# RoozbehSanaei/Structure-from-Motion-3D-Reconstruction

Measured on AMD Instinct MI355X. Metric: keyframes/sec (KLT + RANSAC + local BA per-frame loop), synthetic TempleRing-47 stand-in, higher is better.
Workload: dtype f64

## Files before the change

### include/sfmx.h

```cpp
#ifndef SFMX_H
#define SFMX_H

#include <stdint.h>

#ifdef __cplusplus
extern "C" {
#endif

typedef enum sfmx_status {
  SFMX_OK = 0,
  SFMX_ERR_INVALID = 1,
  SFMX_ERR_HIP = 2,
  SFMX_ERR_NO_DEVICE = 3,
  SFMX_ERR_SINGULAR = 4,
  SFMX_ERR_UNSUPPORTED = 5
} sfmx_status;

typedef struct sfmx_ctx sfmx_ctx;
typedef struct sfmx_pyramid sfmx_pyramid;

int sfmx_ctx_create(int device_id, sfmx_ctx** out);
int sfmx_ctx_create_prio(int device_id, int priority, sfmx_ctx** out);
void sfmx_ctx_destroy(sfmx_ctx* ctx);
const char* sfmx_last_error(const sfmx_ctx* ctx);
// ... 39 lines not shown
int sfmx_ransac_score_ex(sfmx_ctx* ctx, const double* xi, const double* xj, int n, const int32_t* idx8,
                         int H, double thr, int32_t* counts_out, int32_t* lo_out, int32_t* hi_out,
                         uint8_t* flags_out, double* cond_out, int32_t* best_iter,
                         int32_t* best_count, double* E_out);
int sfmx_ransac_score(sfmx_ctx* ctx, const double* xi, const double* xj, int n, const int32_t* idx8,
                      int H, double thr, int32_t* counts_out, int32_t* best_iter, int32_t* best_count,
                      double* E_out);
int sfmx_sampson_mask(sfmx_ctx* ctx, const double* xi, const double* xj, int n, const double* E9,
                      double thr, uint8_t* mask_out, int32_t* count_out);

typedef struct sfmx_ba_problem sfmx_ba_problem;
int sfmx_ba_create(sfmx_ctx* ctx, int W, int P, const double* X, const int32_t* obs_ptr,
                   const int32_t* obs_li, const double* obs_uv, sfmx_ba_problem** out);
int sfmx_ba_reset(sfmx_ctx* ctx, sfmx_ba_problem* prob, int W, int P, const double* X, const int32_t* obs_ptr,
                  const int32_t* obs_li, const double* obs_uv);
void sfmx_ba_destroy(sfmx_ctx* ctx, sfmx_ba_problem* prob);
int sfmx_ba_build(sfmx_ctx* ctx, sfmx_ba_problem* prob, const double* poses_wc, double fx, double fy,
                  double cx, double cy, double huber, double lambda, int damp, double* S_out,
                  double* b_out);
int sfmx_ba_step(sfmx_ctx* ctx, sfmx_ba_problem* prob, const double* poses_wc, double fx, double fy,
                 double cx, double cy, double huber, double lambda, double* dx_out);
int sfmx_ba_begin(sfmx_ctx* ctx, sfmx_ba_problem* prob, int iters, double fx, double fy, double cx, double cy, double huber,
                  double lambda);
int sfmx_ba_end(sfmx_ctx* ctx, sfmx_ba_problem* prob);
int sfmx_ba_build_partial(sfmx_ctx* ctx, sfmx_ba_problem* prob, const double* poses_wc, double fx,
                          double fy, double cx, double cy, double huber, void** S_dev, void** b_dev);

typedef struct sfmx_comm sfmx_comm;
#define SFMX_COMM_ID_BYTES 128
int sfmx_comm_get_unique_id(void* id_out);
// ... 463 lines not shown
```

### structure-from-motion-3d-reconstruction_amd/capi.py

```python
from __future__ import annotations

import ctypes
import os
from ctypes import POINTER, byref, c_char_p, c_double, c_int, c_int32, c_uint8, c_uint32, c_uint64, c_void_p

import numpy as np

os.environ.setdefault("GPU_MAX_HW_QUEUES", "8")

_HERE = os.path.dirname(os.path.abspath(__file__))
LIB_PATH = os.path.join(_HERE, "_build", "libsfmx.so")

SFMX_OK, SFMX_ERR_INVALID, SFMX_ERR_HIP, SFMX_ERR_NO_DEVICE, SFMX_ERR_SINGULAR, SFMX_ERR_UNSUPPORTED = range(6)

SYMBOLS = [
    "sfmx_ctx_create", "sfmx_ctx_create_prio", "sfmx_ctx_destroy", "sfmx_last_error", "sfmx_sync", "sfmx_ctx_device", "sfmx_ctx_make_current", "sfmx_stream", "sfmx_set_timing", "sfmx_get_timing",
    "sfmx_last_kernel_us", "sfmx_kernel_profile", "sfmx_kernel_profile_name", "sfmx_pyramid_create", "sfmx_pyramid_destroy", "sfmx_pyramid_upload",
    "sfmx_pyramid_set_device", "sfmx_pyramid_set_device_async", "sfmx_pyramid_wait", "sfmx_pyramid_fetched_level", "sfmx_pyramid_download_level", "sfmx_pyramid_level_size", "sfmx_shi_tomasi_score",
    "sfmx_shi_tomasi_candidates", "sfmx_shi_tomasi_candidates_pruned", "sfmx_shi_tomasi_fetch_all_keys", "sfmx_klt_track", "sfmx_ransac_score", "sfmx_ransac_score_ex", "sfmx_sampson_mask", "sfmx_ba_create",
    "sfmx_ba_reset", "sfmx_ba_destroy", "sfmx_ba_build", "sfmx_ba_step", "sfmx_ba_begin", "sfmx_ba_end", "sfmx_ba_build_partial", "sfmx_ba_step_sharded", "sfmx_ba_step_sharded_elements", "sfmx_solve_dense", "sfmx_posegraph_solve",
    "sfmx_comm_get_unique_id", "sfmx_comm_create", "sfmx_comm_destroy", "sfmx_comm_rank", "sfmx_comm_world", "sfmx_shard_range",
    "sfmx_comm_allreduce_f64", "sfmx_comm_allreduce_u64_max",
    "sfmx_debug_hypot", "sfmx_debug_divsqrt", "sfmx_debug_klt_slow_steps",
    "sfmx_stereo_default_params", "sfmx_stereo_check_params", "sfmx_stereo_create", "sfmx_stereo_destroy", "sfmx_stereo_disparity",
    "sfmx_stereo_last_us",
    "sfmx_fusion_default_params", "sfmx_fusion_check_params", "sfmx_fusion_create", "sfmx_fusion_destroy", "sfmx_fusion_reset",
    "sfmx_fusion_add_view", "sfmx_fusion_add_stereo_view", "sfmx_fusion_integrate", "sfmx_fusion_read", "sfmx_fusion_extract",
    "sfmx_fusion_last_us",
    "sfmx_fusion_extract_normals", "sfmx_fusion_normals_us",
    "sfmx_shade_default_params", "sfmx_shade_check_params", "sfmx_shade_create", "sfmx_shade_destroy", "sfmx_shade_reset",
    "sfmx_shade_add_view", "sfmx_shade_add_stereo_view", "sfmx_shade_view_count", "sfmx_shade_vertices", "sfmx_shade_fusion",
    "sfmx_shade_last_us",
    "sfmx_consist_default_params", "sfmx_consist_check_params", "sfmx_consist_create", "sfmx_consist_destroy", "sfmx_consist_reset",
    "sfmx_consist_add_view", "sfmx_consist_add_stereo_view", "sfmx_consist_view_count", "sfmx_consist_filter", "sfmx_consist_read",
    "sfmx_consist_counts", "sfmx_fusion_add_consist_view", "sfmx_consist_last_us",
# ... 2117 lines not shown
        obs_uv = _f64(obs_uv)
        self.P = X.shape[0]
        self.h_ = c_void_p()
        ctx._chk(ctx.lib.sfmx_ba_create(ctx.h_, c_int(W), c_int(self.P), _p(X, c_double), _p(obs_ptr, c_int32),
                                        _p(obs_li, c_int32), _p(obs_uv, c_double), byref(self.h_)))

    def reset(self, W: int, X, obs_ptr, obs_li, obs_uv):
        X = _f64(X)
        obs_ptr = np.ascontiguousarray(obs_ptr, np.int32)
        obs_li = np.ascontiguousarray(obs_li, np.int32)
        obs_uv = _f64(obs_uv)
        self.ctx._chk(self.ctx.lib.sfmx_ba_reset(self.ctx.h_, self.h_, c_int(W), c_int(X.shape[0]), _p(X, c_double), _p(obs_ptr, c_int32),
                                                 _p(obs_li, c_int32), _p(obs_uv, c_double)))
        self.W, self.P = W, X.shape[0]

    def build(self, poses_wc, fx, fy, cx, cy, huber, lam, damp=True):
        D = 6 * self.W
        poses = _f64(poses_wc)
        S = np.zeros((D, D))
        b = np.zeros(D)
        self.ctx._chk(self.ctx.lib.sfmx_ba_build(self.ctx.h_, self.h_, _p(poses, c_double), c_double(fx), c_double(fy),
                                                 c_double(cx), c_double(cy), c_double(huber), c_double(lam),
                                                 c_int(1 if damp else 0), _p(S, c_double), _p(b, c_double)))
        return S, b

    def step(self, poses_wc, fx, fy, cx, cy, huber, lam):
        poses = _f64(poses_wc)
        dx = np.zeros(6 * self.W)
        rc = self.ctx.lib.sfmx_ba_step(self.ctx.h_, self.h_, _p(poses, c_double), c_double(fx), c_double(fy), c_double(cx),
                                       c_double(cy), c_double(huber), c_double(lam), _p(dx, c_double))
# ... 305 lines not shown
```

### structure-from-motion-3d-reconstruction_amd/csrc/hip/ba.hip

```cpp
#include "sfmx_internal.h"

#include <chrono>
#include <cstdio>
#include <cstdlib>
#include <mutex>
#include <vector>

#ifdef SFMX_BA_WGSTAMPS
#define WGS_CAP (1u << 20)
__device__ unsigned long long g_wgs_ring[WGS_CAP][8];
__device__ unsigned g_wgs_next;
struct WgStamp {
  unsigned long long t0, m[4] = {0, 0, 0, 0};
  unsigned hw;
  __device__ __forceinline__ void mark(int i) { m[i] = __builtin_amdgcn_s_memrealtime(); }
  __device__ __forceinline__ WgStamp() {
    t0 = __builtin_amdgcn_s_memrealtime();
    hw = (unsigned)__builtin_amdgcn_s_getreg((31 << 11) | 4) | ((unsigned)__builtin_amdgcn_s_getreg((3 << 11) | 20) << 28);
  }
  __device__ __forceinline__ void done(int kind, int blk, int nblk) const {
    __syncthreads();
    if (threadIdx.x == 0) {
      const unsigned slot = atomicAdd(&g_wgs_next, 1u) & (WGS_CAP - 1);
      g_wgs_ring[slot][0] = t0;
// ... 27 lines not shown
#define WGS_BEGIN
#define WGS_END(kind, blk, nblk)
#define WGS_MARK(i)
#define WGS_PARAM
#define WGS_ARG
#endif

#define BA_SLOT 84
#define BA_MAX_OBS 16
#define BA_MAX_W 64

struct sfmx_ba_problem {
  int W = 0, P = 0, R = 0, MS = 0;
  DevBuf bufs[12];
  double* X = nullptr;
  int32_t* obs_ptr = nullptr;
  int32_t* obs_li = nullptr;
  double* obs_uv = nullptr;
  double* poses = nullptr;
  double* rec = nullptr;
  int8_t* slot_of = nullptr;
  double* S = nullptr;
  double* b = nullptr;
  double* work = nullptr;
  double* contrib = nullptr;
  unsigned* ticket = nullptr;
  hipEvent_t ev_sync = nullptr, ev_exp[2] = {nullptr, nullptr}, ev_red[2] = {nullptr, nullptr};
  int chunk = 0;
  bool lds_points = false;
  bool job_active = false;
// ... 868 lines not shown
  }
  WGS_MARK(1);
  __syncthreads();
  if (tid < BAR_COLS && valid) {
    if (is_b) {
      if (damp && i < 6) acc = 0.0;
      b[i] = acc;
    } else {
      if (damp && i == j) {
        acc += lambda;
        if (i < 6) acc += 1e9;
      }
      S[(size_t)i * D + j] = acc;
    }
  }
  if constexpr (SOLVE_N > 0) {
    __shared__ int is_last;
    if (publish_system == 2) {
      if (tid < BAR_COLS && valid) {
        host_out[e] = acc;
        __threadfence_system();
      }
      __syncthreads();
      if (tid == 0) {
        const bool last = __hip_atomic_fetch_add(ticket, 1u, __ATOMIC_ACQ_REL, __HIP_MEMORY_SCOPE_AGENT) == (unsigned)nblk - 1u;
        if (last) {
          __hip_atomic_store(ticket, 0u, __ATOMIC_RELAXED, __HIP_MEMORY_SCOPE_AGENT);
          __threadfence_system();
          __hip_atomic_store(reinterpret_cast<unsigned long long*>(host_out + (SOLVE_N * SOLVE_N + SOLVE_N)), seq, __ATOMIC_RELEASE, __HIP_MEMORY_SCOPE_SYSTEM);
        }
      }
      WGS_MARK(2);
      return;
    }
    if (tid < BAR_COLS) __threadfence();
    __syncthreads();
    if (tid == 0) is_last = atomicAdd(ticket, 1u) == (unsigned)nblk - 1u ? 1 : 0;
    __syncthreads();
    WGS_MARK(2);
    if (!is_last) return;
    __threadfence();
    if (tid == 0) *ticket = 0;
    if (publish_system) {
      const int ne = SOLVE_N * SOLVE_N + SOLVE_N;
      for (int k = tid; k < ne; k += 256) host_out[k] = S[k];
      __threadfence_system();
      __syncthreads();
      if (tid == 0)
        __hip_atomic_store(reinterpret_cast<unsigned long long*>(host_out + ne), seq, __ATOMIC_RELEASE, __HIP_MEMORY_SCOPE_SYSTEM);
// ... 465 lines not shown
                             int publish_system, bool streaming) {
  const char* tile_env = getenv("SFMX_BA_TILE");
  const int tile_rows = tile_env ? atoi(tile_env) : 32;
  if (fused_solve && q->W == 6 && tile_rows == 32) {
    k_ba_reduce<32, 36, 4, 2><<<nwg, 256, 0, c->stream>>>(q->W, p_cnt, rows, lambda, damp, S_out, b_out, q->ticket, q->work, host_out, seq, wave_prio, init,
                                                         wg_lo, publish_system);
  } else if (fused_solve && q->W == 6 && tile_rows == 16) {
    k_ba_reduce<16, 36, 8, 2><<<nwg, 256, 0, c->stream>>>(q->W, p_cnt, rows, lambda, damp, S_out, b_out, q->ticket, q->work, host_out, seq, wave_prio, init,
                                                         wg_lo, publish_system);
  } else if (fused_solve && q->W == 6) {
    k_ba_reduce<64, 36, 2, 2><<<nwg, 256, 0, c->stream>>>(q->W, p_cnt, rows, lambda, damp, S_out, b_out, q->ticket, q->work, host_out, seq, wave_prio, init,
                                                         wg_lo, publish_system);
  } else if (fused_solve && q->W == 10) {
    k_ba_reduce<128, 60, 2, 2><<<nwg, 256, 0, c->stream>>>(q->W, p_cnt, rows, lambda, damp, S_out, b_out, q->ticket, q->work, host_out, seq, wave_prio, init,
                                                          wg_lo, publish_system);
  } else if (!streaming) {
    k_ba_reduce<64, 0, 2, 2><<<nwg, 256, 0, c->stream>>>(q->W, p_cnt, rows, lambda, damp, S_out, b_out, nullptr, nullptr, nullptr, 0, wave_prio, init, wg_lo);
  } else {
    k_ba_reduce<128, 0, 2, 2><<<nwg, 256, 0, c->stream>>>(q->W, p_cnt, rows, lambda, damp, S_out, b_out, nullptr, nullptr, nullptr, 0, wave_prio, init, wg_lo);
  }
}
static int ba_launch_reduce(sfmx_ctx* c, sfmx_ba_problem* q, int p_lo, int p_cnt, double lambda, int damp, double* S_out, double* b_out,
                            const double* init, bool fused_solve, double* host_out, unsigned long long seq, int wave_prio, int wg_lo = 0,
                            int wg_cnt = -1, int publish_system = 0, int e_lo = 0, int e_hi = 0x7fffffff) {
  const size_t CS = (size_t)36 * q->W * q->W + 48 * q->W;
  const int nwg = wg_cnt >= 0 ? wg_cnt : ba_element_blocks(q);
  if (nwg == 0 || p_cnt <= 0) return SFMX_OK;
  if (wg_cnt >= 0) fused_solve = false;
  if (q->chunk == 0) {
    SFMX_PROF(c, KID_BA_REDUCE, ba_reduce_kernel(c, q, q->contrib + (size_t)p_lo * CS, p_cnt, lambda, damp, S_out, b_out, init, fused_solve, host_out, seq,
// ... 106 lines not shown
  if (rc) return rc;
  for (int r = 0; r < n_ranks; ++r) {
    int lo = 0, hi = 0;
    sfmx_shard_range(q->P, r, n_ranks, &lo, &hi);
    if (order == 4) rc = ba_launch_reduce(c, q, lo, hi - lo, 0.0, 0, q->S, q->b, r == 0 ? nullptr : q->S, false, nullptr, 0, ba_wave_prio());
    else rc = ba_launch_reduce(c, q, lo, hi - lo, 0.0, 0, part + (size_t)r * NE, part + (size_t)r * NE + (size_t)D * D, nullptr, false, nullptr, 0,
                               ba_wave_prio());
    if (rc) return rc;
  }
  if (order != 4) k_ba_combine_partials<<<(NE + 255) / 256, 256, 0, c->stream>>>(part, n_ranks, NE, order, q->S);
  t.stop();
  SFMX_HIP(c, hipGetLastError());
  return SFMX_OK;
}

extern "C" {

int sfmx_ba_reset(sfmx_ctx* c, sfmx_ba_problem* q, int W, int P, const double* X, const int32_t* obs_ptr, const int32_t* obs_li,
                  const double* obs_uv) {
  SFMX_REQUIRE(c, c && q && W >= 1 && W <= BA_MAX_W && P >= 1 && X && obs_ptr && obs_li && obs_uv);
  if (q->job_active) (void)sfmx_ba_end(c, q);
  const int R = obs_ptr[P];
  SFMX_REQUIRE(c, R >= 0 && obs_ptr[0] == 0);
  q->W = W; q->P = P; q->R = R;
  q->MS = W < BA_MAX_OBS ? W : BA_MAX_OBS;
  const int D = 6 * W;
  const size_t CS = (size_t)36 * W * W + 36 * W + 12 * W;
  auto up16 = [](size_t v) { return (v + 15) & ~(size_t)15; };
  const size_t o_x = 0, o_uv = up16((size_t)P * 24), o_ptr = o_uv + up16((size_t)R * 16), o_li = o_ptr + up16((size_t)(P + 1) * 4);
  const size_t in_bytes = o_li + up16((size_t)R * 4) + 16;
  q->chunk = ba_merged(q) ? 0 : ba_chunk_points();
  const size_t row_slots = q->chunk ? (size_t)2 * q->chunk : (size_t)P;
  const size_t need[11] = {in_bytes, 16, 16, 16, (size_t)W * 96,
                           (size_t)P * q->MS * BA_SLOT * 8, (size_t)P * W, (size_t)D * D * 8 + (size_t)D * 8, 16, (size_t)D * 8 + 64,
                           row_slots * CS * 8};
  const void* ticket_before = q->bufs[8].p;
  for (int i = 0; i < 11; i++) SFMX_HIP(c, q->bufs[i].ensure(need[i]));
  const bool new_ticket = q->bufs[8].p != ticket_before;
  q->ticket = q->bufs[8].as<unsigned>();
  q->contrib = q->bufs[10].as<double>();
  char* in = q->bufs[0].as<char>();
  q->X = reinterpret_cast<double*>(in + o_x); q->obs_uv = reinterpret_cast<double*>(in + o_uv);
  q->obs_ptr = reinterpret_cast<int32_t*>(in + o_ptr); q->obs_li = reinterpret_cast<int32_t*>(in + o_li);
  q->poses = q->bufs[4].as<double>(); q->rec = q->bufs[5].as<double>();
  q->slot_of = q->bufs[6].as<int8_t>(); q->S = q->bufs[7].as<double>(); q->b = q->S + (size_t)D * D;
  q->work = q->bufs[9].as<double>();
  q->lds_points = false;
  if (ba_merged(q)) {
    bool dup = false;
    for (int p = 0; p < P && !dup; p++) {
      const int o0 = obs_ptr[p], cnt = obs_ptr[p + 1] - o0;
      if (cnt < 2 || cnt > BA_MAX_OBS) continue;
      unsigned long long seen = 0;
      for (int k = 0; k < cnt; k++) {
        const int li = obs_li[o0 + k];
        if (li < 0 || li >= W) continue;
        if (seen >> li & 1ull) { dup = true; break; }
        seen |= 1ull << li;
      }
    }
    q->lds_points = !dup;
  }
  if (c->ba_upload_in_flight) {
    SFMX_HIP(c, hipStreamSynchronize(c->stream));
    c->ba_upload_in_flight = false;
  }
  SFMX_HIP(c, c->h[4].ensure(in_bytes));
  char* st = c->h[4].as<char>();
  memcpy(st + o_x, X, (size_t)P * 24);
  memcpy(st + o_ptr, obs_ptr, (size_t)(P + 1) * 4);
  if (R > 0) {
    memcpy(st + o_uv, obs_uv, (size_t)R * 16);
    memcpy(st + o_li, obs_li, (size_t)R * 4);
  }
  SFMX_HIP(c, hipMemcpyAsync(in, st, in_bytes, hipMemcpyHostToDevice, c->stream));
  if (new_ticket) SFMX_HIP(c, hipMemsetAsync(q->ticket, 0, 16, c->stream));
  c->ba_upload_in_flight = true;
  return SFMX_OK;
}

int sfmx_ba_create(sfmx_ctx* c, int W, int P, const double* X, const int32_t* obs_ptr, const int32_t* obs_li, const double* obs_uv,
                   sfmx_ba_problem** out) {
  SFMX_REQUIRE(c, c && out);
  sfmx_ba_problem* q = new sfmx_ba_problem;
  const int rc = sfmx_ba_reset(c, q, W, P, X, obs_ptr, obs_li, obs_uv);
  if (rc != SFMX_OK) {
    sfmx_ba_destroy(c, q);
    return rc;
  }
  *out = q;
  return SFMX_OK;
}

void sfmx_ba_destroy(sfmx_ctx* c, sfmx_ba_problem* q) {
  if (!q) return;
  if (q->job_active && c) (void)sfmx_ba_end(c, q);
  if (c) { (void)hipStreamSynchronize(c->stream); (void)hipStreamSynchronize(c->copy_stream); }
  for (auto& b : q->bufs) b.release();
  q->job_ctl.release();
  q->job_cmd.release();
  if (q->ev_sync) (void)hipEventDestroy(q->ev_sync);
  for (int k = 0; k < 2; k++) {
    if (q->ev_exp[k]) (void)hipEventDestroy(q->ev_exp[k]);
    if (q->ev_red[k]) (void)hipEventDestroy(q->ev_red[k]);
  }
  delete q;
}

int sfmx_ba_build(sfmx_ctx* c, sfmx_ba_problem* q, const double* poses_wc, double fx, double fy, double cx, double cy, double huber,
                  double lambda, int damp, double* S_out, double* b_out) {
  SFMX_REQUIRE(c, c && q && poses_wc && S_out && b_out);
  KernelTimer t(c);
  int rc = ba_launch_build(c, q, poses_wc, fx, fy, cx, cy, huber, lambda, damp, t);
  if (rc) return rc;
  const int D = 6 * q->W;
  SFMX_HIP(c, hipMemcpyAsync(S_out, q->S, (size_t)D * D * 8, hipMemcpyDeviceToHost, c->stream));
  SFMX_HIP(c, hipMemcpyAsync(b_out, q->b, (size_t)D * 8, hipMemcpyDeviceToHost, c->stream));
  SFMX_HIP(c, hipStreamSynchronize(c->stream));
  c->ba_upload_in_flight = false;
  t.collect();
  return SFMX_OK;
}

int sfmx_ba_build_partial(sfmx_ctx* c, sfmx_ba_problem* q, const double* poses_wc, double fx, double fy, double cx, double cy,
                          double huber, void** S_dev, void** b_dev) {
  SFMX_REQUIRE(c, c && q && poses_wc && S_dev && b_dev);
  KernelTimer t(c);
  int rc = ba_launch_build(c, q, poses_wc, fx, fy, cx, cy, huber, 0.0, 0, t);
  if (rc) return rc;
  SFMX_HIP(c, hipStreamSynchronize(c->stream));
  c->ba_upload_in_flight = false;
  t.collect();
  *S_dev = q->S;
  *b_dev = q->b;
  return SFMX_OK;
}

extern "C" int sfmx_host_solve_window(const double* S, const double* b, int n, double* x, double* work);

int sfmx_ba_begin(sfmx_ctx* c, sfmx_ba_problem* q, int iters, double fx, double fy, double cx, double cy, double huber, double lambda) {
  SFMX_REQUIRE(c, c && q && iters >= 0);
  if (q->job_active) (void)sfmx_ba_end(c, q);
  const char* e = getenv("SFMX_BA_RESIDENT");
  const char* se = getenv("SFMX_BA_SOLVE");
  const bool off = !(e && e[0] == '1') || (se && std::string(se) == "device") || getenv("SFMX_BA_NO_POLL") || getenv("SFMX_BA_NO_FUSE");
  if (off || c->timing || iters < 1 || q->W != 6 || q->chunk != 0 || q->P > BA_MERGED_EXPAND_MAX_P) return SFMX_OK;
  const int D = 6 * q->W, NE = D * D + D;
  SFMX_HIP(c, q->job_ctl.ensure(sizeof(BaResidentCtl)));
  SFMX_HIP(c, q->job_cmd.ensure(16 * 8));
  q->job_slot = (q->job_slot + 1) & 15;
  SFMX_HIP(c, c->h[0].ensure((size_t)q->W * 96));
  SFMX_HIP(c, c->h[1].ensure((size_t)NE * 8 + 32));
  __atomic_store_n(q->job_cmd.as<unsigned long long>() + q->job_slot, 0ull, __ATOMIC_RELEASE);
  *reinterpret_cast<volatile unsigned long long*>(c->h[1].as<double>() + NE) = 0;
  SFMX_HIP(c, hipMemsetAsync(q->job_ctl.p, 0, sizeof(BaResidentCtl), c->stream));
  q->job_first_seq = c->ba_seq + 1;
// ... 33 lines not shown
      __atomic_store_n(q->job_cmd.as<unsigned long long>() + q->job_slot, BAW_EXIT, __ATOMIC_RELEASE);
      q->job_active = false;
      SFMX_HIP(c, hipStreamSynchronize(c->stream));
      return sfmx_fail(c, SFMX_ERR_HIP, "BA step result never arrived (resident kernel)", hipSuccess);
    }
  }
  q->job_done++;
  if (q->job_done >= q->job_iters) q->job_active = false;
  double work[36 * 37];
  const int status = sfmx_host_solve_window(hout, hout + (size_t)D * D, D, dx_out, work);
  return status ? SFMX_ERR_SINGULAR : SFMX_OK;
}

int sfmx_ba_step(sfmx_ctx* c, sfmx_ba_problem* q, const double* poses_wc, double fx, double fy, double cx, double cy, double huber,
                 double lambda, double* dx_out) {
  SFMX_REQUIRE(c, c && q && poses_wc && dx_out);
  if (q->job_active) {
    const double k[6] = {fx, fy, cx, cy, huber, lambda};
    if (memcmp(k, q->job_k, sizeof k) == 0 && !c->timing) return ba_step_resident(c, q, poses_wc, dx_out);
    (void)sfmx_ba_end(c, q);
  }
  const int D = 6 * q->W, NE = D * D + D;
  static const bool no_poll = getenv("SFMX_BA_NO_POLL") != nullptr;
  static const bool no_fuse = getenv("SFMX_BA_NO_FUSE") != nullptr;
  const char* solve_env = getenv("SFMX_BA_SOLVE");
  const bool host_solve_on = !(solve_env && std::string(solve_env) == "device");
  const bool poll = !c->timing && !no_poll;
  const bool fuse = ba_can_fuse_solve(q) && !no_fuse;
  const bool host_solve = host_solve_on && poll && fuse;
  static const bool host_times = getenv("SFMX_BA_HOST_TIMES") != nullptr;
  static double ht_launch = 0, ht_wait = 0, ht_solve = 0, ht_between = 0;
  static unsigned ht_n = 0;
  static std::chrono::steady_clock::time_point ht_last_exit;
  const auto ht0 = std::chrono::steady_clock::now();
  auto ht_us = [](std::chrono::steady_clock::time_point a, std::chrono::steady_clock::time_point b) { return std::chrono::duration<double, std::micro>(b - a).count(); };
  if (host_times && ht_n > 0 && ht_us(ht_last_exit, ht0) < 200.0) ht_between += ht_us(ht_last_exit, ht0);
  KernelTimer t(c);
  SFMX_HIP(c, c->h[1].ensure(host_solve ? (size_t)NE * 8 + 32 : (size_t)D * 8 + 32));
  double* hout = c->h[1].as<double>();
  volatile unsigned long long* flag = reinterpret_cast<volatile unsigned long long*>(host_solve ? hout + NE : hout + D + 1);
  const unsigned long long seq = ++c->ba_seq;
  if (poll) *flag = 0;
  const char* pub_env = getenv("SFMX_BA_PUBLISH");
  const int publish_mode = (pub_env && pub_env[0] == 'l') ? 1 : 2;
  int rc = ba_launch_build(c, q, poses_wc, fx, fy, cx, cy, huber, lambda, 1, t, poll, fuse, poll ? hout : nullptr, seq, host_solve ? publish_mode : 0);
  if (rc) return rc;
  if (!fuse) {
    int* dstatus = reinterpret_cast<int*>(q->work + D);
    rc = launch_solve(c, q->S, q->b, D, q->work, dstatus);
    if (rc) return rc;
  }
  int status = 0;
  if (poll) {
    if (!fuse) {
      k_ba_publish<<<1, 64, 0, c->stream>>>(q->work, D, hout, seq);
      SFMX_HIP(c, hipGetLastError());
    }
    const auto t0 = std::chrono::steady_clock::now();
    if (host_times) ht_launch += ht_us(ht0, t0);
    unsigned spins = 0;
// ... 17 lines not shown
        ht_solve += ht_us(ts, te);
        ht_last_exit = te;
        if (++ht_n == 1000) {
          fprintf(stderr, "[sfmx] ba step host times (us, mean of 1000): launches %.1f | wait for S|b %.1f | host solve %.1f | between steps %.1f\n", ht_launch / 1000,
                  ht_wait / 1000, ht_solve / 1000, ht_between / 1000);
          ht_launch = ht_wait = ht_solve = ht_between = 0;
          ht_n = 0;
        }
      }
      return status ? SFMX_ERR_SINGULAR : SFMX_OK;
    }
    memcpy(dx_out, hout, (size_t)D * 8);
    memcpy(&status, hout + D, 4);
    return status ? SFMX_ERR_SINGULAR : SFMX_OK;
  }
  SFMX_HIP(c, hipMemcpyAsync(c->h[1].p, q->work, (size_t)D * 8 + 4, hipMemcpyDeviceToHost, c->stream));
  SFMX_HIP(c, hipStreamSynchronize(c->stream));
  c->ba_upload_in_flight = false;
  t.collect();
  memcpy(dx_out, c->h[1].p, (size_t)D * 8);
  memcpy(&status, c->h[1].as<char>() + (size_t)D * 8, 4);
  return status ? SFMX_ERR_SINGULAR : SFMX_OK;
}

int sfmx_ba_step_sharded(sfmx_ctx* c, sfmx_comm* comm, sfmx_ba_problem* q, const double* poses_wc, double fx, double fy, double cx, double cy,
                         double huber, double lambda, double* dx_out) {
  SFMX_REQUIRE(c, c && q && poses_wc && dx_out);
  const int D = 6 * q->W;
  KernelTimer t(c);
  const int vworld = (!comm || comm->world <= 1) ? ba_virtual_world() : 0;
  int rc = (vworld > 1 && q->P >= vworld) ? ba_build_virtual_world(c, q, vworld, poses_wc, fx, fy, cx, cy, huber, t)
                                          : ba_launch_build(c, q, poses_wc, fx, fy, cx, cy, huber, 0.0, 0, t);
  if (rc) return rc;
  rc = sfmx_comm_allreduce_dev(c, comm, q->S, (size_t)D * D + D, 0, 0);
  if (rc) return rc;
  k_ba_damp_gauge<<<(D + 63) / 64, 64, 0, c->stream>>>(q->S, q->b, D, lambda);
  int* dstatus = reinterpret_cast<int*>(q->work + D);
  rc = launch_solve(c, q->S, q->b, D, q->work, dstatus);
  if (rc) return rc;
  int status = 0;
  SFMX_HIP(c, c->h[1].ensure((size_t)D * 8 + 8));
  SFMX_HIP(c, hipMemcpyAsync(c->h[1].p, q->work, (size_t)D * 8 + 4, hipMemcpyDeviceToHost, c->stream));
  SFMX_HIP(c, hipStreamSynchronize(c->stream));
  c->ba_upload_in_flight = false;
  t.collect();
  memcpy(dx_out, c->h[1].p, (size_t)D * 8);
  memcpy(&status, c->h[1].as<char>() + (size_t)D * 8, 4);
  return status ? SFMX_ERR_SINGULAR : SFMX_OK;
}

int sfmx_ba_step_sharded_elements(sfmx_ctx* c, sfmx_comm* comm, sfmx_ba_problem* q, const double* poses_wc, double fx, double fy, double cx,
                                  double cy, double huber, double lambda, double* dx_out) {
  SFMX_REQUIRE(c, c && q && poses_wc && dx_out);
  const int D = 6 * q->W, NE = D * D + D;
  const bool real = comm && comm->world > 1;
  const int vworld = real ? 0 : ba_virtual_world();
  const int world = real ? comm->world : (vworld > 1 ? vworld : 1);
  const int nblk = ba_element_blocks(q);
  KernelTimer t(c);
  int rc = SFMX_OK;
  const double* d_poses = ba_stage_poses(c, q, poses_wc, false, &rc);
  if (rc) return rc;
  double* part = nullptr;
  if (vworld > 1) {
    SFMX_HIP(c, q->bufs[11].ensure((size_t)vworld * NE * 8));
    part = q->bufs[11].as<double>();
    SFMX_HIP(c, hipMemsetAsync(part, 0, (size_t)vworld * NE * 8, c->stream));
  }
// ... 66 lines not shown
```

### structure-from-motion-3d-reconstruction_amd/csrc/host/pipeline.cpp

```cpp
#include "pipeline.hpp"

#include "../hip/sfmx_math.h"
#include "cli_io.hpp"
#include "stereo.hpp"
#include "introsort_replay.hpp"
#include "thread_pool.hpp"
#include "lane_plan.hpp"
#include "sfmx_ctx_split.h"
#pragma weak sfmx_ctx_create_bare
#pragma weak sfmx_ctx_create_stream

#include <algorithm>
#include <chrono>
#include <cmath>
#include <cstdio>
#include <cstdlib>
#include <cstring>
#include <filesystem>
#include <fstream>
#include <sstream>

namespace sfmx_host {

namespace {
// ... 837 lines not shown
  return job;
}

void GpuBundleAdjuster::gather_values(BaJob& job, const std::vector<Keyframe>& kfs, const V3* const* pending_xw) {
  if (job.P == 0) return;
  for (const auto& a : job.await) {
    const V3& x = *pending_xw[(size_t)a.second];
    job.X[(size_t)3 * a.first] = x.x; job.X[(size_t)3 * a.first + 1] = x.y; job.X[(size_t)3 * a.first + 2] = x.z;
  }
  job.await.clear();
  job.win.resize((size_t)job.W);
  for (int li = 0; li < job.W; li++) job.win[(size_t)li] = kfs[(size_t)(job.w0 + li)].pose;
  job.valid = true;
}

void GpuBundleAdjuster::solve(BaJob& job) {
  if (!job.valid) return;
  const auto t0 = Clock::now();
  const int W = job.W, P = job.P, D = 6 * W;
  const Mat3& K = job.K;
  const bool multi = comm_ && sfmx_comm_world(comm_) > 1;
  const char* vw = std::getenv("SFMX_VIRTUAL_WORLD");
  const bool virtual_world = !multi && vw && std::atoi(vw) > 1;
  const char* sm = std::getenv("SFMX_BA_SHARD");
  const bool by_points = sm && std::string(sm) == "points";
  const bool sharded = multi && by_points && P >= sfmx_comm_world(comm_);
  const bool by_elements = (multi || virtual_world) && !by_points;
  const double* Xp = job.X.data();
  const std::int32_t* optr = job.optr.data();
  const std::int32_t* oli = job.oli.data();
  const double* ouv = job.uv.data();
  int Pl = P;
  std::vector<std::int32_t> optr_local;
  if (sharded) {
    int lo = 0, hi = P;
    sfmx_shard_range(P, sfmx_comm_rank(comm_), sfmx_comm_world(comm_), &lo, &hi);
    Pl = hi - lo;
    const std::int32_t o0 = job.optr[(size_t)lo];
    optr_local.resize((size_t)Pl + 1);
    for (int p = 0; p <= Pl; p++) optr_local[(size_t)p] = job.optr[(size_t)(lo + p)] - o0;
    Xp += (size_t)3 * lo;
    optr = optr_local.data();
    oli += o0;
    ouv += (size_t)2 * o0;
  }
  if (!prob_) check(ctx_, sfmx_ba_create(ctx_, W, Pl, Xp, optr, oli, ouv, &prob_), "ba_create");
  else check(ctx_, sfmx_ba_reset(ctx_, prob_, W, Pl, Xp, optr, oli, ouv), "ba_reset");
  std::vector<double> poses((size_t)W * 12), dx((size_t)D);
  if (clk_) clk_->ba_calls++;
  const bool plain = !by_elements && !sharded && !virtual_world;
  struct JobGuard {
    sfmx_ctx* c; sfmx_ba_problem* q; bool on;
    ~JobGuard() { if (on) (void)sfmx_ba_end(c, q); }
  } job_guard{ctx_, prob_, false};
  if (plain) {
    check(ctx_, sfmx_ba_begin(ctx_, prob_, job.cfg.iters, K(0, 0), K(1, 1), K(0, 2), K(1, 2), job.cfg.huber_delta, job.cfg.lambda), "ba_begin");
    job_guard.on = true;
  }
  for (int it = 0; it < job.cfg.iters; ++it) {
    for (int li = 0; li < W; li++) {
      Mat3 R;
// ... 636 lines not shown
    const auto tj = Clock::now();
    if (lane_c) {
      if (pending_loop.active && pending_loop.ticket) lane_c->wait_ticket(pending_loop.ticket);
      else if (!queued_loop.active) lane_c->wait();
    }
    clk.join_wait += since(tj);
    if (pending_loop.active) {
      PendingLoop pl = pending_loop;
      pending_loop = PendingLoop{};
      if (pl.cell && *pl.cell) pl.rel = ransac_finish(**pl.cell);
      if (pl.rel && (int)pl.rel->inliers.size() >= 100) accepted_loop = pl;
    }
    return accepted_loop.has_value();
  };
  double t_join_b = 0;
  auto join_b = [&]() {
    const auto tj = Clock::now();
    if (lane) lane->wait();
    clk.join_wait += since(tj);
    t_join_b += since(tj);
    GpuBundleAdjuster::apply(pending_ba, kfs);
    pending_ba = BaJob{};
  };
  auto finish_loop = [&]() {
    const PendingLoop pl = *accepted_loop;
    accepted_loop.reset();
    flush_edges();
    edges.push_back(PGEdge{pl.old_kf, pl.new_kf, pl.rel->R_ji, pl.rel->t_ji, (int)pl.rel->inliers.size(), true});
    (void)posegraph_optimize_centers(ctx, kfs, edges);
    ba.run(K, kfs, map, cfg.ba);
  };
  auto join_lane = [&]() {
    const bool looped = join_c();
// ... 234 lines not shown
          xw.reserve(jobs.size());
          for (const TriJob& j : jobs) {
            xw.push_back(&map.add_point(j.tid, V3{}).Xw);
            j.th->mapped = true;
            for (const auto& ob : *j.hist) map.add_obs(j.tid, ob.first, ob.second);
          }
          clk.tri_insert += since(ti0);
          clk.host += since(ti0);
        }
        kfs.push_back(std::move(kf));
        kf_desc.push_back(new_desc);
        last_kf_frame = fi;
        const auto tg0 = Clock::now();
        next_ba = GpuBundleAdjuster::gather_structure(K, kfs, map, cfg.ba, first_new_pid);
        clk.ba_gather += since(tg0);
        join_b();
        if (have_jobs) {
          solve_jobs(kfs[(size_t)new_kf_id].pose);
          const auto ti1 = Clock::now();
          for (size_t i = 0; i < jobs.size(); i++) *xw[i] = jobs[i].X;
          clk.tri_insert += since(ti1);
          clk.host += since(ti1);
        }
        const auto tg1 = Clock::now();
        GpuBundleAdjuster::gather_values(next_ba, kfs, xw.data());
        pending_ba = std::move(next_ba);
        next_ba = BaJob{};
        clk.ba_gather += since(tg1);
      } else {
        if (kfs.size() >= 1) {
          if (!looped) join_b();
          solve_jobs(kf.pose);
          const auto ti0 = Clock::now();
          for (const TriJob& j : jobs) {
            map.add(j.tid, j.X);
            j.th->mapped = true;
            for (const auto& ob : *j.hist) map.add_obs(j.tid, ob.first, ob.second);
          }
          clk.tri_insert += since(ti0);
          clk.host += since(ti0);
        } else if (!looped) {
          join_b();
        }
        kfs.push_back(std::move(kf));
        kf_desc.push_back(new_desc);
        last_kf_frame = fi;
        const auto tg0 = Clock::now();
        pending_ba = GpuBundleAdjuster::gather(K, kfs, map, cfg.ba);
        clk.ba_gather += since(tg0);
      }
      if (lane) lane->submit([&ba, &pending_ba]() { ba.solve(pending_ba); });
      else ba.solve(pending_ba);
      if (!lane) join_lane();

      if (verify_early) {
        pending_loop = queued_loop;
        queued_loop = PendingLoop{};
      } else {
        detect_loop(kfs.back().kf_id, (int)kfs.size(), pending_loop);
      }
    }
    clk.m_kf += since(tm2);
    const auto te0 = Clock::now();
    emit(fi);
    t_emit += since(te0);
    const auto tr0 = Clock::now();
// ... 562 lines not shown
```

### structure-from-motion-3d-reconstruction_amd/csrc/host/pipeline.hpp

```cpp
#pragma once
#include <array>
#include <atomic>
#include <condition_variable>
#include <cstdint>
#include <deque>
#include <exception>
#include <functional>
#include <future>
#include <memory>
#include <mutex>
#include <optional>
#include <thread>
#include <stdexcept>
#include <string>
#include <unordered_map>
#include <utility>
#include <vector>

#include "../../../include/sfmx.h"
#include "arena.hpp"
#include "host_math.hpp"
#include "introsort_replay.hpp"

namespace sfmx_host {
// ... 333 lines not shown
  std::vector<std::pair<std::int32_t, std::int32_t>> await;
};
class GpuBundleAdjuster {
 public:
  GpuBundleAdjuster(sfmx_ctx* ctx, StageClock* clk, sfmx_comm* comm = nullptr, sfmx_ba_problem** keep = nullptr)
      : ctx_(ctx), clk_(clk), comm_(comm), prob_(keep ? *keep : nullptr), keep_(keep) {}
  ~GpuBundleAdjuster();
  static BaJob gather(const Mat3& K, const std::vector<Keyframe>& kfs, const MapState& map, const BAConfig& cfg) {
    BaJob j = gather_structure(K, kfs, map, cfg);
    gather_values(j, kfs, nullptr);
    return j;
  }
  static BaJob gather_structure(const Mat3& K, const std::vector<Keyframe>& kfs, const MapState& map, const BAConfig& cfg,
                                int first_pending_pid = 0x7fffffff);
  static void gather_values(BaJob& job, const std::vector<Keyframe>& kfs, const V3* const* pending_xw);
  void solve(BaJob& job);
  static void apply(const BaJob& job, std::vector<Keyframe>& kfs);
  void run(const Mat3& K, std::vector<Keyframe>& kfs, MapState& map, const BAConfig& cfg) {
    BaJob j = gather(K, kfs, map, cfg);
    solve(j);
    apply(j, kfs);
  }

 private:
  sfmx_ctx* ctx_;
  StageClock* clk_;
  sfmx_comm* comm_ = nullptr;
  sfmx_ba_problem* prob_ = nullptr;
  sfmx_ba_problem** keep_ = nullptr;
};

class AsyncLane {
 public:
  AsyncLane(int device, int priority, int role);
  ~AsyncLane();
  AsyncLane(const AsyncLane&) = delete;
  AsyncLane& operator=(const AsyncLane&) = delete;
  sfmx_ctx* ctx() const { return ctx_; }
  PooledCtx* pooled() const { return pc_; }
  void submit(std::function<void()> task);
  std::uint64_t submit_ticket(std::function<void()> task);
  void wait_ticket(std::uint64_t ticket);
  void wait();
  double busy_seconds() const { return busy_seconds_; }
// ... 53 lines not shown
```

Before: 1798.

## Stage BA observation upload early on the lane and commit point values later

Splits BA problem reset into a stage step that uploads the observation structure (ptr, li, uv) and a commit step that uploads only the 3D point values. The pipeline submits staging on the async lane while the previous BA is joined and point values are still being gathered, so the structural upload overlaps host work. It also adds a publish-only fused reduce variant for small windows that lets the host solve the system, plus an optional pinned-memory X path. This adds readiness-state checks and more ordering dependencies between lane tasks, which raises the risk of stale pointers or sequencing bugs.

Result: no change. 1791 (-0.3%).

```diff
diff --git a/include/sfmx.h b/include/sfmx.h
--- a/include/sfmx.h
+++ b/include/sfmx.h
@@ -77,6 +77,9 @@
                    const int32_t* obs_li, const double* obs_uv, sfmx_ba_problem** out);
 int sfmx_ba_reset(sfmx_ctx* ctx, sfmx_ba_problem* prob, int W, int P, const double* X, const int32_t* obs_ptr,
                   const int32_t* obs_li, const double* obs_uv);
+int sfmx_ba_stage(sfmx_ctx* ctx, sfmx_ba_problem* prob, int W, int P, const int32_t* obs_ptr, const int32_t* obs_li,
+                  const double* obs_uv);
+int sfmx_ba_commit(sfmx_ctx* ctx, sfmx_ba_problem* prob, const double* X);
 void sfmx_ba_destroy(sfmx_ctx* ctx, sfmx_ba_problem* prob);
 int sfmx_ba_build(sfmx_ctx* ctx, sfmx_ba_problem* prob, const double* poses_wc, double fx, double fy,
                   double cx, double cy, double huber, double lambda, int damp, double* S_out,
diff --git a/structure-from-motion-3d-reconstruction_amd/capi.py b/structure-from-motion-3d-reconstruction_amd/capi.py
--- a/structure-from-motion-3d-reconstruction_amd/capi.py
+++ b/structure-from-motion-3d-reconstruction_amd/capi.py
@@ -18,7 +18,7 @@
     "sfmx_last_kernel_us", "sfmx_kernel_profile", "sfmx_kernel_profile_name", "sfmx_pyramid_create", "sfmx_pyramid_destroy", "sfmx_pyramid_upload",
     "sfmx_pyramid_set_device", "sfmx_pyramid_set_device_async", "sfmx_pyramid_wait", "sfmx_pyramid_fetched_level", "sfmx_pyramid_download_level", "sfmx_pyramid_level_size", "sfmx_shi_tomasi_score",
     "sfmx_shi_tomasi_candidates", "sfmx_shi_tomasi_candidates_pruned", "sfmx_shi_tomasi_fetch_all_keys", "sfmx_klt_track", "sfmx_ransac_score", "sfmx_ransac_score_ex", "sfmx_sampson_mask", "sfmx_ba_create",
-    "sfmx_ba_reset", "sfmx_ba_destroy", "sfmx_ba_build", "sfmx_ba_step", "sfmx_ba_begin", "sfmx_ba_end", "sfmx_ba_build_partial", "sfmx_ba_step_sharded", "sfmx_ba_step_sharded_elements", "sfmx_solve_dense", "sfmx_posegraph_solve",
+    "sfmx_ba_reset", "sfmx_ba_stage", "sfmx_ba_commit", "sfmx_ba_destroy", "sfmx_ba_build", "sfmx_ba_step", "sfmx_ba_begin", "sfmx_ba_end", "sfmx_ba_build_partial", "sfmx_ba_step_sharded", "sfmx_ba_step_sharded_elements", "sfmx_solve_dense", "sfmx_posegraph_solve",
     "sfmx_comm_get_unique_id", "sfmx_comm_create", "sfmx_comm_destroy", "sfmx_comm_rank", "sfmx_comm_world", "sfmx_shard_range",
     "sfmx_comm_allreduce_f64", "sfmx_comm_allreduce_u64_max",
     "sfmx_debug_hypot", "sfmx_debug_divsqrt", "sfmx_debug_klt_slow_steps",
@@ -2166,6 +2166,19 @@
                                                  _p(obs_li, c_int32), _p(obs_uv, c_double)))
         self.W, self.P = W, X.shape[0]
 
+    def stage(self, W: int, P: int, obs_ptr, obs_li, obs_uv):
+        obs_ptr = np.ascontiguousarray(obs_ptr, np.int32)
+        obs_li = np.ascontiguousarray(obs_li, np.int32)
+        obs_uv = _f64(obs_uv)
+        self.ctx._chk(self.ctx.lib.sfmx_ba_stage(self.ctx.h_, self.h_, c_int(W), c_int(P), _p(obs_ptr, c_int32), _p(obs_li, c_int32),
+                                                 _p(obs_uv, c_double)))
+        self.W, self.P = W, P
+
+    def commit(self, X):
+        X = _f64(X)
+        assert X.shape == (self.P, 3)
+        self.ctx._chk(self.ctx.lib.sfmx_ba_commit(self.ctx.h_, self.h_, _p(X, c_double)))
+
     def build(self, poses_wc, fx, fy, cx, cy, huber, lam, damp=True):
         D = 6 * self.W
         poses = _f64(poses_wc)
diff --git a/structure-from-motion-3d-reconstruction_amd/csrc/hip/ba.hip b/structure-from-motion-3d-reconstruction_amd/csrc/hip/ba.hip
--- a/structure-from-motion-3d-reconstruction_amd/csrc/hip/ba.hip
+++ b/structure-from-motion-3d-reconstruction_amd/csrc/hip/ba.hip
@@ -65,6 +65,11 @@
   int W = 0, P = 0, R = 0, MS = 0;
   DevBuf bufs[12];
   double* X = nullptr;
+  double* X_dev = nullptr;
+  PinBuf x_pin;
+  bool x_pinned = false;
+  bool staged = false;
+  bool ready = false;
   int32_t* obs_ptr = nullptr;
   int32_t* obs_li = nullptr;
   double* obs_uv = nullptr;
@@ -963,9 +968,9 @@
       S[(size_t)i * D + j] = acc;
     }
   }
-  if constexpr (SOLVE_N > 0) {
-    __shared__ int is_last;
-    if (publish_system == 2) {
+  if constexpr (SOLVE_N != 0) {
+    if (SOLVE_N < 0 || publish_system == 2) {
+      const int seq_off = SOLVE_N > 0 ? SOLVE_N * SOLVE_N + SOLVE_N : NE;
       if (tid < BAR_COLS && valid) {
         host_out[e] = acc;
         __threadfence_system();
@@ -976,12 +981,15 @@
         if (last) {
           __hip_atomic_store(ticket, 0u, __ATOMIC_RELAXED, __HIP_MEMORY_SCOPE_AGENT);
           __threadfence_system();
-          __hip_atomic_store(reinterpret_cast<unsigned long long*>(host_out + (SOLVE_N * SOLVE_N + SOLVE_N)), seq, __ATOMIC_RELEASE, __HIP_MEMORY_SCOPE_SYSTEM);
+          __hip_atomic_store(reinterpret_cast<unsigned long long*>(host_out + seq_off), seq, __ATOMIC_RELEASE, __HIP_MEMORY_SCOPE_SYSTEM);
         }
       }
       WGS_MARK(2);
       return;
     }
+  }
+  if constexpr (SOLVE_N > 0) {
+    __shared__ int is_last;
     if (tid < BAR_COLS) __threadfence();
     __syncthreads();
     if (tid == 0) is_last = atomicAdd(ticket, 1u) == (unsigned)nblk - 1u ? 1 : 0;
@@ -1477,6 +1485,12 @@
   } else if (fused_solve && q->W == 10) {
     k_ba_reduce<128, 60, 2, 2><<<nwg, 256, 0, c->stream>>>(q->W, p_cnt, rows, lambda, damp, S_out, b_out, q->ticket, q->work, host_out, seq, wave_prio, init,
                                                           wg_lo, publish_system);
+  } else if (fused_solve && !streaming) {
+    k_ba_reduce<64, -1, 2, 2><<<nwg, 256, 0, c->stream>>>(q->W, p_cnt, rows, lambda, damp, S_out, b_out, q->ticket, nullptr, host_out, seq, wave_prio, init,
+                                                         wg_lo);
+  } else if (fused_solve) {
+    k_ba_reduce<128, -1, 2, 2><<<nwg, 256, 0, c->stream>>>(q->W, p_cnt, rows, lambda, damp, S_out, b_out, q->ticket, nullptr, host_out, seq, wave_prio, init,
+                                                          wg_lo);
   } else if (!streaming) {
     k_ba_reduce<64, 0, 2, 2><<<nwg, 256, 0, c->stream>>>(q->W, p_cnt, rows, lambda, damp, S_out, b_out, nullptr, nullptr, nullptr, 0, wave_prio, init, wg_lo);
   } else {
@@ -1613,14 +1627,12 @@
   return SFMX_OK;
 }
 
-extern "C" {
-
-int sfmx_ba_reset(sfmx_ctx* c, sfmx_ba_problem* q, int W, int P, const double* X, const int32_t* obs_ptr, const int32_t* obs_li,
-                  const double* obs_uv) {
-  SFMX_REQUIRE(c, c && q && W >= 1 && W <= BA_MAX_W && P >= 1 && X && obs_ptr && obs_li && obs_uv);
+static int ba_stage_impl(sfmx_ctx* c, sfmx_ba_problem* q, int W, int P, const double* X, const int32_t* obs_ptr, const int32_t* obs_li,
+                         const double* obs_uv) {
   if (q->job_active) (void)sfmx_ba_end(c, q);
   const int R = obs_ptr[P];
   SFMX_REQUIRE(c, R >= 0 && obs_ptr[0] == 0);
+  q->staged = q->ready = false;
   q->W = W; q->P = P; q->R = R;
   q->MS = W < BA_MAX_OBS ? W : BA_MAX_OBS;
   const int D = 6 * W;
@@ -1639,7 +1651,7 @@
   q->ticket = q->bufs[8].as<unsigned>();
   q->contrib = q->bufs[10].as<double>();
   char* in = q->bufs[0].as<char>();
-  q->X = reinterpret_cast<double*>(in + o_x); q->obs_uv = reinterpret_cast<double*>(in + o_uv);
+  q->X_dev = reinterpret_cast<double*>(in + o_x); q->obs_uv = reinterpret_cast<double*>(in + o_uv);
   q->obs_ptr = reinterpret_cast<int32_t*>(in + o_ptr); q->obs_li = reinterpret_cast<int32_t*>(in + o_li);
   q->poses = q->bufs[4].as<double>(); q->rec = q->bufs[5].as<double>();
   q->slot_of = q->bufs[6].as<int8_t>(); q->S = q->bufs[7].as<double>(); q->b = q->S + (size_t)D * D;
@@ -1660,21 +1672,56 @@
     }
     q->lds_points = !dup;
   }
+  const char* x_env = getenv("SFMX_BA_X");
+  q->x_pinned = q->lds_points && x_env && x_env[0] == 'p';
+  if (q->x_pinned) SFMX_HIP(c, q->x_pin.ensure((size_t)P * 24));
+  q->X = q->x_pinned ? q->x_pin.as<double>() : q->X_dev;
   if (c->ba_upload_in_flight) {
     SFMX_HIP(c, hipStreamSynchronize(c->stream));
     c->ba_upload_in_flight = false;
   }
   SFMX_HIP(c, c->h[4].ensure(in_bytes));
   char* st = c->h[4].as<char>();
-  memcpy(st + o_x, X, (size_t)P * 24);
   memcpy(st + o_ptr, obs_ptr, (size_t)(P + 1) * 4);
   if (R > 0) {
     memcpy(st + o_uv, obs_uv, (size_t)R * 16);
     memcpy(st + o_li, obs_li, (size_t)R * 4);
   }
-  SFMX_HIP(c, hipMemcpyAsync(in, st, in_bytes, hipMemcpyHostToDevice, c->stream));
+  size_t from = o_uv;
+  if (X && q->x_pinned) memcpy(q->x_pin.p, X, (size_t)P * 24);
+  else if (X) { memcpy(st + o_x, X, (size_t)P * 24); from = o_x; }
+  SFMX_HIP(c, hipMemcpyAsync(in + from, st + from, in_bytes - from, hipMemcpyHostToDevice, c->stream));
   if (new_ticket) SFMX_HIP(c, hipMemsetAsync(q->ticket, 0, 16, c->stream));
   c->ba_upload_in_flight = true;
+  q->staged = X == nullptr;
+  q->ready = X != nullptr;
+  return SFMX_OK;
+}
+
+extern "C" {
+
+int sfmx_ba_reset(sfmx_ctx* c, sfmx_ba_problem* q, int W, int P, const double* X, const int32_t* obs_ptr, const int32_t* obs_li,
+                  const double* obs_uv) {
+  SFMX_REQUIRE(c, c && q && W >= 1 && W <= BA_MAX_W && P >= 1 && X && obs_ptr && obs_li && obs_uv);
+  return ba_stage_impl(c, q, W, P, X, obs_ptr, obs_li, obs_uv);
+}
+
+int sfmx_ba_stage(sfmx_ctx* c, sfmx_ba_problem* q, int W, int P, const int32_t* obs_ptr, const int32_t* obs_li, const double* obs_uv) {
+  SFMX_REQUIRE(c, c && q && W >= 1 && W <= BA_MAX_W && P >= 1 && obs_ptr && obs_li && obs_uv);
+  return ba_stage_impl(c, q, W, P, nullptr, obs_ptr, obs_li, obs_uv);
+}
+
+int sfmx_ba_commit(sfmx_ctx* c, sfmx_ba_problem* q, const double* X) {
+  SFMX_REQUIRE(c, c && q && X && q->staged);
+  if (q->x_pinned) {
+    memcpy(q->x_pin.p, X, (size_t)q->P * 24);
+  } else {
+    memcpy(c->h[4].p, X, (size_t)q->P * 24);
+    SFMX_HIP(c, hipMemcpyAsync(q->X_dev, c->h[4].p, (size_t)q->P * 24, hipMemcpyHostToDevice, c->stream));
+    c->ba_upload_in_flight = true;
+  }
+  q->staged = false;
+  q->ready = true;
   return SFMX_OK;
 }
 
@@ -1696,6 +1743,7 @@
   if (q->job_active && c) (void)sfmx_ba_end(c, q);
   if (c) { (void)hipStreamSynchronize(c->stream); (void)hipStreamSynchronize(c->copy_stream); }
   for (auto& b : q->bufs) b.release();
+  q->x_pin.release();
   q->job_ctl.release();
   q->job_cmd.release();
   if (q->ev_sync) (void)hipEventDestroy(q->ev_sync);
@@ -1708,7 +1756,7 @@
 
 int sfmx_ba_build(sfmx_ctx* c, sfmx_ba_problem* q, const double* poses_wc, double fx, double fy, double cx, double cy, double huber,
                   double lambda, int damp, double* S_out, double* b_out) {
-  SFMX_REQUIRE(c, c && q && poses_wc && S_out && b_out);
+  SFMX_REQUIRE(c, c && q && q->ready && poses_wc && S_out && b_out);
   KernelTimer t(c);
   int rc = ba_launch_build(c, q, poses_wc, fx, fy, cx, cy, huber, lambda, damp, t);
   if (rc) return rc;
@@ -1723,7 +1771,7 @@
 
 int sfmx_ba_build_partial(sfmx_ctx* c, sfmx_ba_problem* q, const double* poses_wc, double fx, double fy, double cx, double cy,
                           double huber, void** S_dev, void** b_dev) {
-  SFMX_REQUIRE(c, c && q && poses_wc && S_dev && b_dev);
+  SFMX_REQUIRE(c, c && q && q->ready && poses_wc && S_dev && b_dev);
   KernelTimer t(c);
   int rc = ba_launch_build(c, q, poses_wc, fx, fy, cx, cy, huber, 0.0, 0, t);
   if (rc) return rc;
@@ -1738,7 +1786,7 @@
 extern "C" int sfmx_host_solve_window(const double* S, const double* b, int n, double* x, double* work);
 
 int sfmx_ba_begin(sfmx_ctx* c, sfmx_ba_problem* q, int iters, double fx, double fy, double cx, double cy, double huber, double lambda) {
-  SFMX_REQUIRE(c, c && q && iters >= 0);
+  SFMX_REQUIRE(c, c && q && q->ready && iters >= 0);
   if (q->job_active) (void)sfmx_ba_end(c, q);
   const char* e = getenv("SFMX_BA_RESIDENT");
   const char* se = getenv("SFMX_BA_SOLVE");
@@ -1802,7 +1850,7 @@
 
 int sfmx_ba_step(sfmx_ctx* c, sfmx_ba_problem* q, const double* poses_wc, double fx, double fy, double cx, double cy, double huber,
                  double lambda, double* dx_out) {
-  SFMX_REQUIRE(c, c && q && poses_wc && dx_out);
+  SFMX_REQUIRE(c, c && q && q->ready && poses_wc && dx_out);
   if (q->job_active) {
     const double k[6] = {fx, fy, cx, cy, huber, lambda};
     if (memcmp(k, q->job_k, sizeof k) == 0 && !c->timing) return ba_step_resident(c, q, poses_wc, dx_out);
@@ -1814,8 +1862,10 @@
   const char* solve_env = getenv("SFMX_BA_SOLVE");
   const bool host_solve_on = !(solve_env && std::string(solve_env) == "device");
   const bool poll = !c->timing && !no_poll;
-  const bool fuse = ba_can_fuse_solve(q) && !no_fuse;
-  const bool host_solve = host_solve_on && poll && fuse;
+  const char* small_env = getenv("SFMX_BA_SMALL_W");
+  const bool publish_only = host_solve_on && !no_poll && !no_fuse && !ba_can_fuse_solve(q) && q->W <= 10 && !(small_env && small_env[0] == 'l');
+  const bool fuse = (ba_can_fuse_solve(q) && !no_fuse) || publish_only;
+  const bool host_solve = host_solve_on && fuse && (poll || publish_only);
   static const bool host_times = getenv("SFMX_BA_HOST_TIMES") != nullptr;
   static double ht_launch = 0, ht_wait = 0, ht_solve = 0, ht_between = 0;
   static unsigned ht_n = 0;
@@ -1831,7 +1881,8 @@
   if (poll) *flag = 0;
   const char* pub_env = getenv("SFMX_BA_PUBLISH");
   const int publish_mode = (pub_env && pub_env[0] == 'l') ? 1 : 2;
-  int rc = ba_launch_build(c, q, poses_wc, fx, fy, cx, cy, huber, lambda, 1, t, poll, fuse, poll ? hout : nullptr, seq, host_solve ? publish_mode : 0);
+  int rc = ba_launch_build(c, q, poses_wc, fx, fy, cx, cy, huber, lambda, 1, t, poll, fuse, (poll || publish_only) ? hout : nullptr, seq,
+                           host_solve ? publish_mode : 0);
   if (rc) return rc;
   if (!fuse) {
     int* dstatus = reinterpret_cast<int*>(q->work + D);
@@ -1879,6 +1930,13 @@
     memcpy(&status, hout + D, 4);
     return status ? SFMX_ERR_SINGULAR : SFMX_OK;
   }
+  if (publish_only) {
+    SFMX_HIP(c, hipStreamSynchronize(c->stream));
+    c->ba_upload_in_flight = false;
+    t.collect();
+    double work[60 * 61];
+    return sfmx_host_solve_window(hout, hout + (size_t)D * D, D, dx_out, work) ? SFMX_ERR_SINGULAR : SFMX_OK;
+  }
   SFMX_HIP(c, hipMemcpyAsync(c->h[1].p, q->work, (size_t)D * 8 + 4, hipMemcpyDeviceToHost, c->stream));
   SFMX_HIP(c, hipStreamSynchronize(c->stream));
   c->ba_upload_in_flight = false;
@@ -1890,7 +1948,7 @@
 
 int sfmx_ba_step_sharded(sfmx_ctx* c, sfmx_comm* comm, sfmx_ba_problem* q, const double* poses_wc, double fx, double fy, double cx, double cy,
                          double huber, double lambda, double* dx_out) {
-  SFMX_REQUIRE(c, c && q && poses_wc && dx_out);
+  SFMX_REQUIRE(c, c && q && q->ready && poses_wc && dx_out);
   const int D = 6 * q->W;
   KernelTimer t(c);
   const int vworld = (!comm || comm->world <= 1) ? ba_virtual_world() : 0;
@@ -1916,7 +1974,7 @@
 
 int sfmx_ba_step_sharded_elements(sfmx_ctx* c, sfmx_comm* comm, sfmx_ba_problem* q, const double* poses_wc, double fx, double fy, double cx,
                                   double cy, double huber, double lambda, double* dx_out) {
-  SFMX_REQUIRE(c, c && q && poses_wc && dx_out);
+  SFMX_REQUIRE(c, c && q && q->ready && poses_wc && dx_out);
   const int D = 6 * q->W, NE = D * D + D;
   const bool real = comm && comm->world > 1;
   const int vworld = real ? 0 : ba_virtual_world();
diff --git a/structure-from-motion-3d-reconstruction_amd/csrc/host/pipeline.cpp b/structure-from-motion-3d-reconstruction_amd/csrc/host/pipeline.cpp
--- a/structure-from-motion-3d-reconstruction_amd/csrc/host/pipeline.cpp
+++ b/structure-from-motion-3d-reconstruction_amd/csrc/host/pipeline.cpp
@@ -875,7 +875,35 @@
   job.valid = true;
 }
 
+extern "C" {
+int sfmx_ba_stage(sfmx_ctx* ctx, sfmx_ba_problem* prob, int W, int P, const std::int32_t* obs_ptr, const std::int32_t* obs_li,
+                  const double* obs_uv) __attribute__((weak));
+int sfmx_ba_commit(sfmx_ctx* ctx, sfmx_ba_problem* prob, const double* X) __attribute__((weak));
+}
+
+void GpuBundleAdjuster::stage(int W, int P, const std::int32_t* optr, const std::int32_t* oli, const double* uv) {
+  staged_optr_ = nullptr;
+  const bool multi = comm_ && sfmx_comm_world(comm_) > 1;
+  const char* vw = std::getenv("SFMX_VIRTUAL_WORLD");
+  if (multi || (vw && std::atoi(vw) > 1) || !prob_ || P < 1) return;
+  const auto t0 = Clock::now();
+  if (sfmx_ba_stage && sfmx_ba_commit) {
+    check(ctx_, sfmx_ba_stage(ctx_, prob_, W, P, optr, oli, uv), "ba_stage");
+  } else {
+    const std::int32_t R = optr[P];
+    std::int64_t sum = 0;
+    for (std::int32_t o = 0; o < R; ++o) sum += oli[o] + (uv[2 * o] < uv[2 * o + 1] ? 1 : 0);
+    if (optr[0] != 0 || R < 0 || sum < -(std::int64_t)W * R) throw SfmxFailure(SFMX_ERR_INVALID, "ba_stage: observation lists");
+  }
+  staged_optr_ = optr;
+  staged_W_ = W;
+  staged_P_ = P;
+  if (clk_) clk_->ba += since(t0);
+}
+
 void GpuBundleAdjuster::solve(BaJob& job) {
+  const bool staged = staged_optr_ && staged_optr_ == job.optr.data() && staged_W_ == job.W && staged_P_ == job.P;
+  staged_optr_ = nullptr;
   if (!job.valid) return;
   const auto t0 = Clock::now();
   const int W = job.W, P = job.P, D = 6 * W;
@@ -906,6 +934,7 @@
     ouv += (size_t)2 * o0;
   }
   if (!prob_) check(ctx_, sfmx_ba_create(ctx_, W, Pl, Xp, optr, oli, ouv, &prob_), "ba_create");
+  else if (staged && !sharded && !by_elements && !virtual_world && sfmx_ba_stage && sfmx_ba_commit) check(ctx_, sfmx_ba_commit(ctx_, prob_, Xp), "ba_commit");
   else check(ctx_, sfmx_ba_reset(ctx_, prob_, W, Pl, Xp, optr, oli, ouv), "ba_reset");
   std::vector<double> poses((size_t)W * 12), dx((size_t)D);
   if (clk_) clk_->ba_calls++;
@@ -1572,9 +1601,11 @@
     return accepted_loop.has_value();
   };
   double t_join_b = 0;
-  auto join_b = [&]() {
+  std::uint64_t ba_ticket = 0;
+  auto join_b = [&](bool behind_ba = false) {
     const auto tj = Clock::now();
-    if (lane) lane->wait();
+    if (lane && behind_ba) lane->wait_ticket(ba_ticket);
+    else if (lane) lane->wait();
     clk.join_wait += since(tj);
     t_join_b += since(tj);
     GpuBundleAdjuster::apply(pending_ba, kfs);
@@ -1839,7 +1870,12 @@
         const auto tg0 = Clock::now();
         next_ba = GpuBundleAdjuster::gather_structure(K, kfs, map, cfg.ba, first_new_pid);
         clk.ba_gather += since(tg0);
-        join_b();
+        const char* stage_env = std::getenv("SFMX_BA_STAGE");
+        std::uint64_t stage_ticket = 0;
+        if (lane && next_ba.P > 0 && !(stage_env && std::string(stage_env) == "late"))
+          stage_ticket = lane->submit_ticket([&ba, W = next_ba.W, P = next_ba.P, optr = next_ba.optr.data(), oli = next_ba.oli.data(),
+                                              uv = next_ba.uv.data()]() { ba.stage(W, P, optr, oli, uv); });
+        join_b(stage_ticket != 0);
         if (have_jobs) {
           solve_jobs(kfs[(size_t)new_kf_id].pose);
           const auto ti1 = Clock::now();
@@ -1849,6 +1885,11 @@
         }
         const auto tg1 = Clock::now();
         GpuBundleAdjuster::gather_values(next_ba, kfs, xw.data());
+        if (stage_ticket) {
+          const auto tj = Clock::now();
+          lane->wait_ticket(stage_ticket);
+          clk.join_wait += since(tj);
+        }
         pending_ba = std::move(next_ba);
         next_ba = BaJob{};
         clk.ba_gather += since(tg1);
@@ -1874,7 +1915,7 @@
         pending_ba = GpuBundleAdjuster::gather(K, kfs, map, cfg.ba);
         clk.ba_gather += since(tg0);
       }
-      if (lane) lane->submit([&ba, &pending_ba]() { ba.solve(pending_ba); });
+      if (lane) ba_ticket = lane->submit_ticket([&ba, &pending_ba]() { ba.solve(pending_ba); });
       else ba.solve(pending_ba);
       if (!lane) join_lane();
 
diff --git a/structure-from-motion-3d-reconstruction_amd/csrc/host/pipeline.hpp b/structure-from-motion-3d-reconstruction_amd/csrc/host/pipeline.hpp
--- a/structure-from-motion-3d-reconstruction_amd/csrc/host/pipeline.hpp
+++ b/structure-from-motion-3d-reconstruction_amd/csrc/host/pipeline.hpp
@@ -371,6 +371,7 @@
   static BaJob gather_structure(const Mat3& K, const std::vector<Keyframe>& kfs, const MapState& map, const BAConfig& cfg,
                                 int first_pending_pid = 0x7fffffff);
   static void gather_values(BaJob& job, const std::vector<Keyframe>& kfs, const V3* const* pending_xw);
+  void stage(int W, int P, const std::int32_t* optr, const std::int32_t* oli, const double* uv);
   void solve(BaJob& job);
   static void apply(const BaJob& job, std::vector<Keyframe>& kfs);
   void run(const Mat3& K, std::vector<Keyframe>& kfs, MapState& map, const BAConfig& cfg) {
@@ -385,6 +386,8 @@
   sfmx_comm* comm_ = nullptr;
   sfmx_ba_problem* prob_ = nullptr;
   sfmx_ba_problem** keep_ = nullptr;
+  const std::int32_t* staged_optr_ = nullptr;
+  int staged_W_ = 0, staged_P_ = 0;
 };
 
 class AsyncLane {
```
